# ChanganVR/RelationalGraphLearning

Hardware: AMD Instinct MI355X
Metric: agent-graph forward evals/sec (N=20, 2-layer GCN, depth-2 tree) (higher is better)
Workload: dtype f32 (24-bit operands throughout; 13 312 of the 14 224 products of the children kernel's 32 x 32, 32 x 100 and 100 x 100 head matrices, its embedding / graph weight products (w_r's second layer, Wa, W1, W_last) and the state predictor's weight products as six bf16 MFMA terms over three round-to-neare

## Files before the change

### relationalgraphlearning_amd/csrc/rgl_fused.hip

```cpp
#include "rgl_mlp_chain.h"
#include "rgl_scene_body.h"
#include "rgl_tail.h"

#include <mutex>
#include <unordered_map>
#include <vector>

namespace {

__host__ __device__ constexpr bool fused_packed_rows(int HR, bool SOFT) { return SOFT && HR <= 20; }
__host__ __device__ constexpr int fused_scratch_floats(int HR, int NT, bool SOFT) {
    const int NP = 16 * NT, HRL = HR < NP ? HR : NP;
    const int main_fl = fused_packed_rows(HR, SOFT) ? HRL * 32 + 16 * (HRL + 2) * 2 : 2 * 16 * (NP + 1) + 16 * XLD;
    const int crowd_fl = NP * XLD + 2 * NP;
    const int fl = main_fl > crowd_fl ? main_fl : crowd_fl;
    return ((fl > kTailLdsInts ? fl : kTailLdsInts) + 3) & ~3;
}

struct FusedArgs {
    const float *wr1, *br1, *wr2, *br2, *wa, *w1;
    const float *wh1, *bh1, *wh2, *bh2;
    const float* w_last;
    const float *hw1, *hb1, *hw2, *hb2, *hw3, *hb3, *hw4, *hb4;
    const float* child_robot;
// ... 237 lines not shown
                    xt[nt][ot][r] = Xs[(16 * nt + 4 * q + r) * XLD + 16 * ot + n];
        if constexpr (T1P) {
#pragma unroll
            for (int ot = 0; ot < 2; ++ot) xt1p[ot] = Xs[(16 + q) * XLD + 16 * ot + n];
        }
        load_fence();
        __builtin_amdgcn_wave_barrier();
        
        Split3 xqs[BX ? NT : 1], xts[BX ? 2 : 1];
        if constexpr (BX) {
            static_assert(NT <= 2, "Xh^T: one chunk over the nodes");
#pragma unroll
            for (int jt = 0; jt < NT; ++jt) xqs[jt] = split3_pair(xq[jt][0], xq[jt][1]);
            if constexpr (BXS) xpc[0] = xqs[0];
#pragma unroll
            for (int ft = 0; ft < 2; ++ft) xts[ft] = split3_pair(xt[0][ft], NT > 1 ? xt[NT > 1 ? 1 : 0][ft] : zero4());
        }
#pragma unroll
        for (int pct = 0; pct < NT; ++pct) {
            const int node = 16 * pct + n;
            const bool node_ok = node >= 1 && node < N;
            f32x4 e[NT];
            float mx = NEG_INF;
            Split3 gs;
            if constexpr (BX) {
                gs = split3_pair(gq[pct][0], gq[pct][1]);
                if (BXS && pct == 0) gpc[0] = gs;
            }
#pragma unroll
            for (int jt = 0; jt < NT; ++jt) {
                f32x4 sacc = zero4();
                if constexpr (BX) sacc = b6_block(xqs[jt], gs, sacc);
                else {
#pragma unroll
                for (int ft = 0; ft < 2; ++ft)
#pragma unroll
                    for (int r = 0; r < 4; ++r) sacc = mfma4(xq[jt][ft][r], gq[pct][ft][r], sacc);
                }
#pragma unroll
                for (int r = 0; r < 4; ++r) {
                    const int j = 16 * jt + 4 * q + r;
                    if (sim != SIM_SOFTMAX) sacc[r] = plain_weight(sim, sacc[r], node, j);
                    if (j < 1 || j >= N) sacc[r] = sim == SIM_SOFTMAX ? NEG_INF : 0.f;
                    mx = fmaxf(mx, sacc[r]);
                }
                e[jt] = sacc;
            }
            mx = kgroups_max(mx);
            if (!node_ok || sim != SIM_SOFTMAX) mx = 0.f;
            float z = 0.f;
#pragma unroll
            for (int jt = 0; jt < NT; ++jt)
#pragma unroll
                for (int r = 0; r < 4; ++r) {
                    if (sim == SIM_SOFTMAX) e[jt][r] = __expf(e[jt][r] - mx);
                    if (!node_ok) e[jt][r] = 0.f;
                    z += e[jt][r];
                }
            z = kgroups_sum(z);
            if (q == 0) {
                msz[node] = mx;
                msz[NP + node] = node_ok ? z : 1.f;
            }
            f32x4 u[2] = {zero4(), zero4()};
            f32x4 uw[2] = {zero4(), zero4()};
            {
            if constexpr (BX) {
                const Split3 es = split3_pair(e[0], NT > 1 ? e[NT > 1 ? 1 : 0] : zero4());
                u[0] = b6_block(xts[0], es, u[0]);
                u[1] = b6_block(xts[1], es, u[1]);
            } else {
#pragma unroll
            for (int jt = 0; jt < NT; ++jt)
#pragma unroll
                for (int r = 0; r < 4; ++r) {
                    u[0] = mfma4(xt[jt][0][r], e[jt][r], u[0]);
                    u[1] = mfma4(xt[jt][1][r], e[jt][r], u[1]);
                }
            }
            if constexpr (BX) layer_mfma_b6<XD, XD, false>(w1, u, uw, lane);
            else {
#pragma unroll
            for (int ft = 0; ft < 2; ++ft) {
                load_fence();
#pragma unroll
                for (int r = 0; r < 4; ++r)
#pragma unroll
                    for (int ot = 0; ot < 2; ++ot)
                        uw[ot] = mfma4(w1[(16 * ft + 4 * q + r) * WLD + 16 * ot + n], u[ft][r], uw[ot]);
            }
            load_fence();
            }
            }
            if constexpr (PK) {
                if (node < HRL) {
                    *reinterpret_cast<f32x4*>(&UWs[node * 32 + 4 * q]) = uw[0];
                    *reinterpret_cast<f32x4*>(&UWs[node * 32 + 16 + 4 * q]) = uw[1];
                }
            } else {
                *reinterpret_cast<f32x4*>(&Xs[node * XLD + 4 * q]) = uw[0];
                *reinterpret_cast<f32x4*>(&Xs[node * XLD + 16 + 4 * q]) = uw[1];
            }
        }
        __builtin_amdgcn_wave_barrier();
        load_fence();
#pragma unroll
        for (int nt = 0; nt < (T1P ? 1 : NT); ++nt) {
            ms[nt] = *reinterpret_cast<const f32x4*>(&msz[16 * nt + 4 * q]);
            zs[nt] = *reinterpret_cast<const f32x4*>(&msz[NP + 16 * nt + 4 * q]);
        }
        if constexpr (T1P) {
            ms1 = msz[16 + q];
            zs1 = msz[NP + 16 + q];
#pragma unroll
            for (int ot = 0; ot < 2; ++ot)
#pragma unroll
                for (int r = 0; r < 4; ++r) {
                    gq[1][ot][r] = quad0_bcast(gq[1][ot][r]);
                    xq[1][ot][r] = quad0_bcast(xq[1][ot][r]);
                }
        }
        if constexpr (!PK) {
#pragma unroll
            for (int i4 = 0; i4 < HRL / 4; ++i4)
#pragma unroll
                for (int k = 0; k < 4; ++k) uw4[i4][k] = Xs[(4 * i4 + k) * XLD + (lane & 31)];
        }
        load_fence();
        __builtin_amdgcn_wave_barrier();
    };
    static_assert(LO::scratch % 4 == 0 && LO::f_last % 4 == 0, "b128 granules");
    constexpr int kChunk = 256;
    constexpr int kChunksA = (LO::f_last + kChunk - 1) / kChunk, kChunksAll = (LO::scratch + kChunk - 1) / kChunk;
    int* image_arrivals = reinterpret_cast<int*>(lds + LO::scratch + kFusedWaves * fused_scratch_floats(HR, NT, SOFT));
    auto image_chunk = [&](int c) {
        const int fl = c * kChunk + lane * 4;
        if (fl < LO::scratch)
            __builtin_amdgcn_global_load_lds((const __attribute__((address_space(1))) void*)(a.image + fl),
                                             (__attribute__((address_space(3))) void*)(lds + c * kChunk), 16, 0, 0);
    };
    if constexpr (PRO) {
        static_assert(kPrologueSceneBase<LO> == kChunksA * kChunk, "the scene region starts behind the first part's chunks");
        static_assert(kPrologueSceneBase<LO> + prologue_scene_floats(2, 19) <= LO::scratch + kFusedWaves * fused_scratch_floats(HR, NT, SOFT) + 4,
                      "a two-layer predictor's scene region with the row buffer of a full chunk (12 crowds of 19 humans, 16 robot rows) fits the kernel's LDS");
        ProPhases pro_phases;
        ProPhases* const pp = &pro_phases;
        PRO_PHASE_START(pp);
        for (int c = wave; c < kChunksA; c += kFusedWaves) image_chunk(c);
#ifdef RGL_PROLOGUE_EMB_PER_WAVE
        constexpr bool kWge = false;
#else
        constexpr bool kWge = true;
#endif
        scene_body<2, 0, kFusedWaves, false, true, true, kWge>(pa.scene, lds + kPrologueSceneBase<LO>, p_first, 1, kFusedWaves,
                                                               p_first + k_b, pp);
        const ChildrenArgs& ca = pa.children;
        const long long pair0 = (long long)p_first * ca.A, pair_end = (long long)(p_first + k_b) * ca.A;
        if (ca.A >= 64 && ca.H <= 64 && !ca.robot64) {
            const float v_max = table_speed_bound(ca);
            for (long long base = pair0 + 64 * wave; base < pair_end; base += 64 * kFusedWaves) children_wave(ca, base, pair_end, v_max);
        } else {
            for (long long idx = pair0 + tid; idx < pair_end; idx += nthreads) children_thread(ca, idx);
        }
        PRO_PHASE_MARK(pp, 3);
        __syncthreads();
        PRO_PHASE_MARK(pp, 4);
        PRO_PHASE_FLUSH(pp);
        wh2_loads();
    }
    if (wave < n_items) item_loads(item_at(0));
    if (tid == 0) *image_arrivals = 0;
    bool image_complete = false;
    if (a.image_sync) {
        copy_image<LO::scratch, nthreads>(lds, a.image, tid);
        __syncthreads();
        image_complete = true;
    } else {
    if (!PRO) for (int c = wave; c < kChunksA; c += kFusedWaves) image_chunk(c);
    __builtin_amdgcn_s_waitcnt(0x0F70);
    __syncthreads();
    for (int c = kChunksA + wave; c < kChunksAll; c += kFusedWaves) image_chunk(c);
    }
    auto await_image = [&]() {
        if (image_complete) return;
        __builtin_amdgcn_s_waitcnt(0x0F70);
        asm volatile("" ::: "memory");
        if (lane == 0) __hip_atomic_fetch_add(image_arrivals, 1, __ATOMIC_RELEASE, __HIP_MEMORY_SCOPE_WORKGROUP);
        while (__hip_atomic_load(image_arrivals, __ATOMIC_ACQUIRE, __HIP_MEMORY_SCOPE_WORKGROUP) < kFusedWaves) __builtin_amdgcn_s_sleep(1);
        asm volatile("" ::: "memory");
        image_complete = true;
    };
    if (wave >= 4) {
        for (int i = 0; i < a.phase_delay; ++i) __builtin_amdgcn_s_sleep(8);
        if (a.prio & 1) __builtin_amdgcn_s_setprio(1);
    }
    PHASE_START();
    for (int pass = 0; pass < n_pass; ++pass) {
        const int wi = item_at(pass);
        if (wi >= n_items) break;
        const int wi_next = pass + 1 < n_pass ? item_at(pass + 1) : n_items;
        PHASE_MARK(0);
        int p, t0, ts, t1;
        item_tiles(wi, p, t0, ts, t1);
        load_fence();
        crowd_compute();
        PHASE_MARK(1);

      for (int ti = ts; ti < t1; ++ti) {
        const int t = ti < t0 ? a.n_full : ti;
        const bool full = t < a.n_full;
        const int c = 16 * t + n;
        const int n_valid = full ? 16 : a.rem;

        f32x4 xacc[2] = {zero4(), zero4()}, gacc[2] = {zero4(), zero4()}, yacc[2] = {zero4(), zero4()};
        float s00 = 0.f;
        Split3 sx;
        {
            f32x4 hacc[4] = {zero4(), zero4(), zero4(), zero4()};
#pragma unroll
            for (int s = 0; s < 3; ++s) {
                const int k = 4 * s + q;
#pragma unroll
                for (int ht = 0; ht < 4; ++ht) hacc[ht] = mfma4(wr1[(k < LO::WR1ROWS ? k : LO::WR1ROWS - 1) * LO::WR1LD + 16 * ht + n], rin[s], hacc[ht]);
            }
            if (ti + 1 < t1) robot_rows(p, ti + 1);
#pragma unroll
            for (int ht = 0; ht < 4; ++ht) {
                const f32x4 bb = *reinterpret_cast<const f32x4*>(&br1[16 * ht + 4 * q]);
#pragma unroll
                for (int r = 0; r < 4; ++r) hacc[ht][r] = relu1(hacc[ht][r] + bb[r]);
            }
            if constexpr (BX) {
                layer_mfma_b6<HID, XD, true>(wr2, hacc, xacc, lane, br2);
#pragma unroll
                for (int ot = 0; ot < 2; ++ot)
#pragma unroll
                    for (int r = 0; r < 4; ++r) xacc[ot][r] = relu1(xacc[ot][r]);
                sx = split3_pair(xacc[0], xacc[1]);
                layer_mfma_b6_pre<XD, false>(wa, sx, gacc, lane);
                layer_mfma_b6_pre<XD, false>(w1, sx, yacc, lane);
            } else {
#pragma unroll
            for (int ht = 0; ht < 4; ++ht) {
                load_fence();
#pragma unroll
                for (int r = 0; r < 4; ++r)
#pragma unroll
                    for (int ot = 0; ot < 2; ++ot)
                        xacc[ot] = mfma4(wr2[(16 * ht + 4 * q + r) * WLD + 16 * ot + n], hacc[ht][r], xacc[ot]);
            }
            load_fence();
#pragma unroll
            for (int ot = 0; ot < 2; ++ot) {
                const f32x4 bb = *reinterpret_cast<const f32x4*>(&br2[16 * ot + 4 * q]);
#pragma unroll
                for (int r = 0; r < 4; ++r) xacc[ot][r] = relu1(xacc[ot][r] + bb[r]);
            }
#pragma unroll
            for (int ot = 0; ot < 2; ++ot) {
                load_fence();
#pragma unroll
                for (int r = 0; r < 4; ++r)
#pragma unroll
                    for (int gt = 0; gt < 2; ++gt) {
                        gacc[gt] = mfma4(wa[(16 * ot + 4 * q + r) * WLD + 16 * gt + n], xacc[ot][r], gacc[gt]);
                        yacc[gt] = mfma4(w1[(16 * ot + 4 * q + r) * WLD + 16 * gt + n], xacc[ot][r], yacc[gt]);
                    }
            }
            load_fence();
            }
            if constexpr (!PK) {
                *reinterpret_cast<f32x4*>(&Y0[n * XLD + 4 * q]) = yacc[0];
                *reinterpret_cast<f32x4*>(&Y0[n * XLD + 16 + 4 * q]) = yacc[1];
            }
#pragma unroll
            for (int tt = 0; tt < 2; ++tt)
#pragma unroll
                for (int r = 0; r < 4; ++r) s00 = fmaf(gacc[tt][r], xacc[tt][r], s00);
            s00 = kgroups_sum(s00);
        }

        PHASE_MARK(2);
        f32x4 t0h[2] = {zero4(), zero4()};
        float p00;
        {
            f32x4 s0t[NT], sct[NT];
            float mx0 = NEG_INF;
            float sc1 = NEG_INF, p1 = NEG_INF;
            if constexpr (T1P) {
                f32x4 psc[2] = {zero4(), zero4()}, ps0[2] = {zero4(), zero4()};
#pragma unroll
                for (int ot = 0; ot < 2; ++ot)
#pragma unroll
                    for (int r = 0; r < 4; ++r) {
                        psc[r & 1] = mfma4x4(gq[1][ot][r], xacc[ot][r], psc[r & 1]);
                        ps0[r & 1] = mfma4x4(xq[1][ot][r], gacc[ot][r], ps0[r & 1]);
                    }
                sc1 = kgroups_reduce_scatter(psc[0] + psc[1]);
                p1 = kgroups_reduce_scatter(ps0[0] + ps0[1]);
                if (16 + q >= N) { sc1 = NEG_INF; p1 = NEG_INF; }
                mx0 = p1;
            }
            Split3 sg;
            if constexpr (BXS) sg = split3_pair(gacc[0], gacc[1]);
#pragma unroll
            for (int nt = 0; nt < NTS; ++nt) {
                f32x4 sc = zero4(), s0 = zero4();
// ... 751 lines not shown
```

### relationalgraphlearning_amd/csrc/rgl_mlp_chain.h

```cpp
#pragma once
#include "rgl_mfma.h"

namespace {

template <int D>
struct Tiles { static constexpr int v = (D + 15) / 16; };

template <int D>
__device__ __forceinline__ int tile_feature(int t, int q, int r) {
    constexpr bool partial = (D % 16) != 0;
    return (partial && t == Tiles<D>::v - 1) ? 16 * t + 4 * r + q : 16 * t + 4 * q + r;
}
template <int D>
struct LastTileSteps { static constexpr int v = (D % 16) == 0 ? 4 : ((D % 16) + 3) / 4; };

template <int OUT>
struct Partial4 { static constexpr bool v = (OUT % 16) != 0 && (OUT % 16) <= 4; };
template <int OUT>
__device__ __forceinline__ int frag_out_feature(int ot, int l) {
    if (Partial4<OUT>::v && ot == Tiles<OUT>::v - 1) return 16 * ot + (l & 3);
    const int m = l & 15;
    return tile_feature<OUT>(ot, m >> 2, m & 3);
}
template <int IN, int OUT, int NTHR = 0>
// ... 361 lines not shown
        constexpr int cn = (st + 1) / NP, prn = (st + 1) % NP;
        __builtin_amdgcn_sched_barrier(0);
        if constexpr (WB == 2 && has_next) {
#pragma unroll
            for (int g = 0; g < 2; ++g)
#pragma unroll
                for (int pc = 0; pc < 3; ++pc) w[WB == 2 ? buf ^ 1 : 0][g][pc] = frag_at(cn, 2 * prn + g, pc);
        }
        if constexpr (WB == 1) {
#pragma unroll
            for (int g = 0; g < 2; ++g)
#pragma unroll
                for (int pc = 0; pc < 3; ++pc) w[0][g][pc] = frag_at(c, 2 * pr + g, pc);
        }
        const bf16x8 sh = __builtin_bit_cast(bf16x8, u32x4{H[0], H[1], H[2], H[3]}), sm = __builtin_bit_cast(bf16x8, u32x4{M[0], M[1], M[2], M[3]}),
                     sl = __builtin_bit_cast(bf16x8, u32x4{L[0], L[1], L[2], L[3]});
#define RGL_BX_TERM(WP, AP)                                                                                         \
    _Pragma("unroll") for (int g = 0; g < 2; ++g)                                                                   \
        out[2 * pr + g] = __builtin_amdgcn_mfma_f32_16x16x32_bf16(w[buf][g][WP], AP, out[2 * pr + g], 0, 0, 0);
        RGL_BX_TERM(2, sh)
        RGL_BX_TERM(1, sm)
        RGL_BX_TERM(0, sl)
        RGL_BX_TERM(1, sh)
        RGL_BX_TERM(0, sm)
        RGL_BX_TERM(0, sh)
#undef RGL_BX_TERM
        if constexpr (c + 1 < NC) {
            constexpr int u0 = (4 * pr) / NP, u1 = (4 * (pr + 1)) / NP;
            static_for<u0, u1>([&](auto uc) {
                constexpr int p = decltype(uc)::value;
                split3_unit(unit_of(c + 1, p), Hn_[p], Mn_[p], Ln_[p]);
            });
        }
        if constexpr (WB == 1) __builtin_amdgcn_sched_group_barrier(0x100, 6, 0);
        __builtin_amdgcn_sched_group_barrier(0x008, 1, 0);
        if constexpr (WB == 2) __builtin_amdgcn_sched_group_barrier(0x100, has_next ? 6 : 0, 0);
#pragma unroll
        for (int i = 0; i < 11; ++i) {
            __builtin_amdgcn_sched_group_barrier(0x002, 2, 0);
            __builtin_amdgcn_sched_group_barrier(0x008, 1, 0);
        }
        if constexpr (pr == NP - 1 && c + 1 < NC) {
#pragma unroll
            for (int p = 0; p < 4; ++p) { H[p] = Hn_[p]; M[p] = Mn_[p]; L[p] = Ln_[p]; }
        }
    });
    __builtin_amdgcn_sched_barrier(0);
#pragma unroll
    for (int it = ITB + (BL::OT3 > 0 ? 2 : 0); it < IT; ++it) {
        load_fence();
#pragma unroll
        for (int r = 0; r < 4; ++r) {
            if (it == IT - 1 && r >= LastTileSteps<IN>::v) continue;
#pragma unroll
            for (int ot = 0; ot < OTF; ++ot) {
                const int k = (it - ITB - (ot < BL::OT3 ? 2 : 0)) * 4 + r;
                out[ot] = mfma4(fl[BL::f32_of(ot) + k * 64], in[it][r], out[ot]);
            }
        }
    }
    load_fence();
    if constexpr (BL::P4) out[OTF] = f32x4{v4, 0.f, 0.f, 0.f};
}

template <int IN, int OUT, bool BIAS>
__device__ __forceinline__ void layer_mfma_bx1(const float* frags, const f32x4 (&in)[Tiles<IN>::v], f32x4 (&out)[Tiles<OUT>::v],
                                               int lane, const float* bias = nullptr) {
    using BL = Bx1Layout<IN, OUT>;
    constexpr int OTF = BL::OTF;
    const int q = lane >> 4;
    float v4 = 0.f;
    if constexpr (BL::P4) {
        v4 = partial4_compact<IN, BL::KP>(frags + BL::p4, in, lane);
        if constexpr (BIAS) v4 += bias[16 * OTF + 4 * q];
    }
#pragma unroll
    for (int ot = 0; ot < OTF; ++ot) {
        if constexpr (BIAS) out[ot] = *reinterpret_cast<const f32x4*>(&bias[16 * ot + 4 * q]);
        else out[ot] = zero4();
    }
    load_fence();
    const Split3 s = split3_pair(in[0], in[1]);
    constexpr int G = 2;
#pragma unroll
    for (int o0 = 0; o0 < OTF; o0 += G) {
        load_fence();
        bf16x8 w[G][3];
#pragma unroll
        for (int g = 0; g < G; ++g)
#pragma unroll
            for (int pc = 0; pc < 3; ++pc)
                if (o0 + g < OTF) w[g][pc] = *reinterpret_cast<const bf16x8*>(&frags[BL::b16 + (((o0 + g) * 3 + pc) * 64 + lane) * 4]);
#define RGL_BX_TERM(WP, AP)                                                                                         \
    _Pragma("unroll") for (int g = 0; g < G; ++g)                                                                   \
        if (o0 + g < OTF) out[o0 + g] = __builtin_amdgcn_mfma_f32_16x16x32_bf16(w[g][WP], s.AP, out[o0 + g], 0, 0, 0);
        RGL_BX_TERM(2, h)
        RGL_BX_TERM(1, m)
        RGL_BX_TERM(0, l)
        RGL_BX_TERM(1, h)
        RGL_BX_TERM(0, m)
        RGL_BX_TERM(0, h)
#undef RGL_BX_TERM
    }
    load_fence();
    if constexpr (BL::P4) out[OTF] = f32x4{v4, 0.f, 0.f, 0.f};
}

template <int IN, int OUT>
struct B6Floats { static constexpr int v = Tiles<OUT>::v * ((Tiles<IN>::v + 1) / 2) * 3 * 64 * 4; };

template <int IN, int OUT, bool BIAS>
__device__ __forceinline__ void layer_mfma_b6(const float* frags, const f32x4 (&in)[Tiles<IN>::v], f32x4 (&out)[Tiles<OUT>::v],
                                              int lane, const float* bias = nullptr) {
    constexpr int IT = Tiles<IN>::v, OT = Tiles<OUT>::v, NC = (IT + 1) / 2;
    static_assert(IN % 16 == 0, "full input tiles");
    const int q = lane >> 4;
#pragma unroll
    for (int ot = 0; ot < OT; ++ot) {
        if constexpr (BIAS) out[ot] = *reinterpret_cast<const f32x4*>(&bias[16 * ot + 4 * q]);
        else out[ot] = zero4();
    }
    constexpr int G = 2, NOB = (OT + G - 1) / G, NB = NC * NOB;
    bf16x8 w[2][G][3];
    auto load_block = [&](int b, int buf) {
        const int c = b / NOB, o0 = G * (b % NOB);
#pragma unroll
        for (int g = 0; g < G; ++g)
#pragma unroll
            for (int pc = 0; pc < 3; ++pc)
                if (o0 + g < OT) w[buf][g][pc] = *reinterpret_cast<const bf16x8*>(&frags[((((o0 + g) * NC + c) * 3 + pc) * 64 + lane) * 4]);
    };
    load_fence();
    load_block(0, 0);
    Split3 s;
    static_for<0, NB>([&](auto bc) {
        constexpr int b = decltype(bc)::value, c = b / NOB, o0 = G * (b % NOB), buf = b & 1;
        if constexpr (b % NOB == 0) s = split3_pair(in[2 * c], 2 * c + 1 < IT ? in[2 * c + 1 < IT ? 2 * c + 1 : 0] : zero4());
        load_fence();
        if constexpr (b + 1 < NB) load_block(b + 1, buf ^ 1);
#define RGL_B6_TERM(WP, AP)                                                                                         \
    _Pragma("unroll") for (int g = 0; g < G; ++g)                                                                   \
        if (o0 + g < OT) out[o0 + g] = __builtin_amdgcn_mfma_f32_16x16x32_bf16(w[buf][g][WP], s.AP, out[o0 + g], 0, 0, 0);
        RGL_B6_TERM(2, h)
        RGL_B6_TERM(1, m)
        RGL_B6_TERM(0, l)
        RGL_B6_TERM(1, h)
        RGL_B6_TERM(0, m)
        RGL_B6_TERM(0, h)
#undef RGL_B6_TERM
    });
    load_fence();
}

template <int OUT, bool BIAS>
__device__ __forceinline__ void layer_mfma_b6_pre(const float* frags, const Split3& s, f32x4 (&out)[Tiles<OUT>::v], int lane,
                                                  const float* bias = nullptr) {
    constexpr int OT = Tiles<OUT>::v;
    const int q = lane >> 4;
#pragma unroll
    for (int ot = 0; ot < OT; ++ot) {
        if constexpr (BIAS) out[ot] = *reinterpret_cast<const f32x4*>(&bias[16 * ot + 4 * q]);
        else out[ot] = zero4();
    }
    constexpr int G = 2;
#pragma unroll
    for (int o0 = 0; o0 < OT; o0 += G) {
        load_fence();
        bf16x8 w[G][3];
#pragma unroll
        for (int g = 0; g < G; ++g)
#pragma unroll
            for (int pc = 0; pc < 3; ++pc)
                if (o0 + g < OT) w[g][pc] = *reinterpret_cast<const bf16x8*>(&frags[(((o0 + g) * 3 + pc) * 64 + lane) * 4]);
#define RGL_B6_TERM(WP, AP)                                                                                         \
    _Pragma("unroll") for (int g = 0; g < G; ++g)                                                                   \
        if (o0 + g < OT) out[o0 + g] = __builtin_amdgcn_mfma_f32_16x16x32_bf16(w[g][WP], s.AP, out[o0 + g], 0, 0, 0);
        RGL_B6_TERM(2, h)
        RGL_B6_TERM(1, m)
        RGL_B6_TERM(0, l)
        RGL_B6_TERM(1, h)
        RGL_B6_TERM(0, m)
        RGL_B6_TERM(0, h)
#undef RGL_B6_TERM
    }
    load_fence();
}

template <int IN, int OUT>
__device__ __forceinline__ float frag_bf3_ld(const float* __restrict__ W, int ld, int n_out, int idx) {
    constexpr int IT = Tiles<IN>::v, NC = (IT + 1) / 2;
    const int u = idx >> 2, p = idx & 3;
    const int l = u & 63, rest = u >> 6;
    const int pc = rest % 3, c = (rest / 3) % NC, ot = rest / 3 / NC;
    const int m = l & 15, q = l >> 4;
    const int out = 16 * ot + m;
    bf16x2 v;
#pragma unroll
    for (int k = 0; k < 2; ++k) {
        const int e = 2 * p + k, t = 2 * c + (e >> 2);
        const int in = 16 * t + 4 * q + (e & 3);
        const float w = (t < IT && in < IN && out < n_out) ? W[in * ld + out] : 0.f;
        const __bf16 hi = (__bf16)w;
        const float r1 = w - (float)hi;
        const __bf16 mid = (__bf16)r1;
        const __bf16 lo = (__bf16)(r1 - (float)mid);
        v[k] = pc == 0 ? hi : (pc == 1 ? mid : lo);
    }
    return __builtin_bit_cast(float, v);
}

template <int D>
__device__ __forceinline__ float frag_bf3_identity(int idx) {
    constexpr int IT = Tiles<D>::v, NC = (IT + 1) / 2;
    const int u = idx >> 2, p = idx & 3;
    const int l = u & 63, rest = u >> 6;
    const int pc = rest % 3, c = (rest / 3) % NC, ot = rest / 3 / NC;
    bf16x2 v;
#pragma unroll
    for (int k = 0; k < 2; ++k) {
        const int e = 2 * p + k, in = 16 * (2 * c + (e >> 2)) + 4 * (l >> 4) + (e & 3), out = 16 * ot + (l & 15);
        v[k] = (__bf16)((pc == 0 && in == out) ? 1.f : 0.f);
    }
    return __builtin_bit_cast(float, v);
}

template <int OUT>
__device__ __forceinline__ void relu_tiles(f32x4 (&x)[Tiles<OUT>::v]) {
#pragma unroll
    for (int ot = 0; ot < Tiles<OUT>::v; ++ot)
#pragma unroll
        for (int r = 0; r < 4; ++r) x[ot][r] = relu1(x[ot][r]);
}

}
```

### relationalgraphlearning_amd/csrc/rgl_scene_body.h

```cpp
#pragma once
#include "rgl_children.h"
#include "rgl_mlp_chain.h"

using rgl::LevelPrologue;
using rgl::SceneArgs;

namespace {

constexpr int M2LD = 20;

constexpr int kPrologueChunk = 16, kPrologueChunkCrowds = 12;
__host__ __device__ inline int prologue_chunk_end(int c0, int end, int crowds_per, int max_crowds) {
    int c1 = c0 + kPrologueChunk;
    const int by_crowds = (c0 / crowds_per + max_crowds) * crowds_per;
    if (by_crowds < c1) c1 = by_crowds;
    return c1 < end ? c1 : end;
}
constexpr int prologue_row_floats(int H, int max_crowds) { return (max_crowds * H + kPrologueChunk) * XD; }

struct SceneImageLayout { int off_wa, off_ws, off_wm1, off_bm1, off_wm2, off_bm2, total, ws_stride; };
constexpr SceneImageLayout scene_image_layout(int L, bool bx = false) {
    SceneImageLayout o{};
    int off = 0;
    auto take = [&](int nfl) { int r = off; off += (nfl + 3) & ~3; return r; };
    o.ws_stride = bx ? B6Floats<XD, XD>::v : XD * WLD;
    o.off_wa = take(bx ? B6Floats<XD, XD>::v : XD * WLD);
    o.off_ws = take(L * o.ws_stride);
    o.off_wm1 = take(bx ? B6Floats<XD, HID>::v : XD * W1LD);
    o.off_bm1 = take(HID);
    o.off_wm2 = take(bx ? B6Floats<HID, 16>::v : HID * M2LD);
    o.off_bm2 = take(16);
    o.total = off;
    return o;
}

constexpr int kRowMlpSetFloats = 4 * 1 * 4 * 64 + 2 * 4 * 4 * 64 + HID + XD;
constexpr int prologue_scene_floats(int L, int H) {
    return scene_image_layout(L, true).total + 2 * kRowMlpSetFloats + 8 * 32 * XLD + prologue_row_floats(H, kPrologueChunkCrowds);
}

#ifdef RGL_PHASE_TIMING
struct ProPhases { unsigned long long acc[5] = {0, 0, 0, 0, 0}, t0 = 0; };
#define PRO_PHASE_START(pp) do { if (pp) (pp)->t0 = __builtin_amdgcn_s_memtime(); } while (0)
#define PRO_PHASE_MARK(pp, idx)                                            \
    do {                                                                   \
        if (pp) {                                                          \
            const unsigned long long now__ = __builtin_amdgcn_s_memtime(); \
            (pp)->acc[idx] += now__ - (pp)->t0;                            \
            (pp)->t0 = now__;                                              \
        }                                                                  \
    } while (0)
#define PRO_PHASE_FLUSH(pp)                                                \
    do {                                                                   \
        if ((threadIdx.x & 63) == 0)                                       \
            for (int i__ = 0; i__ < 5; ++i__) atomicAdd(&g_phase_cycles[10 + i__], (pp)->acc[i__]); \
    } while (0)
#else
struct ProPhases {};
#define PRO_PHASE_START(pp) do { } while (0)
#define PRO_PHASE_MARK(pp, idx) do { } while (0)
#define PRO_PHASE_FLUSH(pp) do { (void)(pp); } while (0)
#endif

template <int IN>
__device__ __forceinline__ void row_mlp2_tile(const float* lds_set, const float* src, int lane, f32x4 (&o)[2]) {
    constexpr int F1 = 0, F2 = F1 + 4 * 1 * 4 * 64, B1 = F2 + 2 * 4 * 4 * 64, B2 = B1 + HID;
    const int q = lane >> 4;
    f32x4 in[1];
#pragma unroll
    for (int r = 0; r < 4; ++r) {
        const int feat = tile_feature<IN>(0, q, r);
        in[0][r] = feat < IN ? src[feat] : 0.f;
    }
    f32x4 h[4];
    layer_mfma<IN, HID, true>(lds_set + F1, in, h, lane, lds_set + B1);
    relu_tiles<HID>(h);
    layer_mfma<HID, XD, true>(lds_set + F2, h, o, lane, lds_set + B2);
    relu_tiles<XD>(o);
}


template <int NT, int SK, int WAVES, bool SPLIT, bool EMB = false, bool BX = false, bool WGE = false>
__device__ __forceinline__ void scene_body(const SceneArgs& a, float* lds, int first, int slot_step, int pass_step, int end,
                                           ProPhases* pp = nullptr) {
    static_assert(!BX || SK == 0, "six-term bf16 products: softmax similarity");
    static_assert(!WGE || (EMB && !SPLIT), "workgroup-cooperative embeddings: the embedding sets in LDS, one scene per wave");
    static_assert(!SPLIT || (SK != 3 && NT > 1 && WAVES % NT == 0), "split scenes: whole scenes per workgroup, no pair-MLP similarity");
    constexpr int kSceneThreads = WAVES * 64;
    constexpr int NCT = SPLIT ? 1 : NT;
    const int sim = SK == 0 ? (int)SIM_SOFTMAX : a.sim;
    const int tid = threadIdx.x, lane = tid & 63, wave = tid >> 6;
    const int n = lane & 15, q = lane >> 4;
    const int N = a.N, H = a.H;
    const float* wa = lds + a.off_wa;
    const float* ws = lds + a.off_ws;
    const float* wm1 = lds + a.off_wm1;
    const float* bm1 = lds + a.off_bm1;
    const float* wm2 = lds + a.off_wm2;
    const float* bm2 = lds + a.off_bm2;
    const int slot = __builtin_amdgcn_readfirstlane(SPLIT ? wave / NT : wave);
    const int ctb = SPLIT ? __builtin_amdgcn_readfirstlane(wave % NT) : 0;
    float* Hs = lds + a.off_wave + slot * a.wave_stride;
    constexpr int kEmbThreads = EMB ? kSceneThreads : 64;
    FragRegs<9, HID, kEmbThreads> er1;
    FragRegs<HID, XD, kEmbThreads> er2, eh2;
    FragRegs<5, HID, kEmbThreads> eh1;
    float ebias[4] = {0.f, 0.f, 0.f, 0.f};
    auto emb_loads = [&]() {
        if constexpr (EMB) {
            frag_load(er1, a.er_w1, tid);
            frag_load(er2, a.er_w2, tid);
            frag_load(eh1, a.eh_w1, tid);
            frag_load(eh2, a.eh_w2, tid);
            ebias[0] = bias_load<HID>(a.er_b1, tid);
            ebias[1] = bias_load<XD>(a.er_b2, tid);
            ebias[2] = bias_load<HID>(a.eh_b1, tid);
            ebias[3] = bias_load<XD>(a.eh_b2, tid);
        }
    };
    if constexpr (BX) {
        constexpr int kChunk = 256;
        const int n_chunks = (a.image_floats + kChunk - 1) / kChunk;
        for (int c = wave; c < n_chunks; c += WAVES) {
            const int fl = c * kChunk + lane * 4;
            if (fl < a.image_floats)
                __builtin_amdgcn_global_load_lds((const __attribute__((address_space(1))) void*)(a.image + fl),
                                                 (__attribute__((address_space(3))) void*)(lds + c * kChunk), 16, 0, 0);
        }
        __builtin_amdgcn_s_waitcnt(0x0F70);
    } else
    {
        float* w = lds;
        constexpr int NT_ = kSceneThreads;
        constexpr int KQ = XD * XD / NT_, KM1 = XD * HID / NT_, KM2 = HID * 16 / NT_;
        float vq[5][KQ];
        float vm1[KM1], vm2[KM2], vb;
        const int Lc = a.L < 4 ? a.L : 4;
#pragma unroll
        for (int k = 0; k < KQ; ++k) {
            const int i = tid + k * NT_;
            vq[0][k] = a.wa ? a.wa[i] : ((i / XD) == (i % XD) ? 1.f : 0.f);
#pragma unroll
            for (int l = 0; l < 4; ++l) vq[1 + l][k] = l < Lc ? a.Ws[l][i] : 0.f;
        }
#pragma unroll
        for (int k = 0; k < KM1; ++k) vm1[k] = a.wm1 ? a.wm1[tid + k * NT_] : 0.f;
#pragma unroll
        for (int k = 0; k < KM2; ++k) {
            const int i = tid + k * NT_, r = i / 16, c = i - r * 16;
            vm2[k] = a.wm2 ? a.wm2[r * 5 + (c < 5 ? c : 0)] : 0.f;
        }
        vb = !a.bm1 ? 0.f : (tid < HID ? a.bm1[tid] : (tid < HID + 5 ? a.bm2[tid - HID] : 0.f));
        emb_loads();
#pragma unroll
        for (int k = 0; k < KQ; ++k) {
            const int i = tid + k * NT_, r = i / XD, c = i - r * XD;
            w[a.off_wa + r * WLD + c] = vq[0][k];
#pragma unroll
            for (int l = 0; l < 4; ++l)
                if (l < Lc) w[a.off_ws + (l * XD + r) * WLD + c] = vq[1 + l][k];
        }
#pragma unroll
        for (int k = 0; k < KM1; ++k) {
            const int i = tid + k * NT_, r = i / HID, c = i - r * HID;
            w[a.off_wm1 + r * W1LD + c] = vm1[k];
        }
#pragma unroll
        for (int k = 0; k < KM2; ++k) {
            const int i = tid + k * NT_, r = i / 16, c = i - r * 16;
            w[a.off_wm2 + r * M2LD + c] = c < 5 ? vm2[k] : 0.f;
        }
        if (tid < HID) w[a.off_bm1 + tid] = vb;
        else if (tid < HID + 16) w[a.off_bm2 + tid - HID] = tid < HID + 5 ? vb : 0.f;
        if (SK == 3) {
            fill_matrix<2 * XD, 2 * XD, HID, W1LD, kSceneThreads>(w + a.off_wc1, a.wc1, tid);
            for (int i = tid; i < HID; i += kSceneThreads) { w[a.off_bc1 + i] = a.bc1[i]; w[a.off_wc2 + i] = a.wc2[i]; }
        }
    }
    if constexpr (EMB) {
        float* w = lds;
        constexpr int F1 = 0, F2 = F1 + 4 * 1 * 4 * 64, B1 = F2 + 2 * 4 * 4 * 64, B2 = B1 + HID;
        if constexpr (BX) emb_loads();
        frag_store(er1, w + a.off_er + F1, tid);
        frag_store(er2, w + a.off_er + F2, tid);
        bias_store<HID>(ebias[0], w + a.off_er + B1, tid);
        bias_store<XD>(ebias[1], w + a.off_er + B2, tid);
        frag_store(eh1, w + a.off_eh + F1, tid);
        frag_store(eh2, w + a.off_eh + F2, tid);
        bias_store<HID>(ebias[2], w + a.off_eh + B1, tid);
        bias_store<XD>(ebias[3], w + a.off_eh + B2, tid);
    }
    __syncthreads();
    PRO_PHASE_MARK(pp, 0);
    if (WGE && first >= end) return;
    int c0 = first;
    do {
    const int c1 = WGE ? prologue_chunk_end(c0, end, a.crowds_per, a.chunk_crowds) : end;
    const int cr0 = WGE ? c0 / a.crowds_per : 0;
    const int robot_rows0 = WGE ? a.off_rows + a.chunk_crowds * H * XD : 0;
    if constexpr (WGE) {
        if (c0 != first) {
            __syncthreads();
            PRO_PHASE_MARK(pp, 4);
        }
        const int hrows = ((c1 - 1) / a.crowds_per - cr0 + 1) * H, htiles = (hrows + 15) >> 4;
        for (int t = wave; t <= htiles; t += WAVES) {
            f32x4 o[2];
            int dst;
            bool valid;
            if (t < htiles) {
                const int row = 16 * t + n;
                valid = row < hrows;
                row_mlp2_tile<5>(lds + a.off_eh, a.human_rows + ((size_t)cr0 * H + (valid ? row : hrows - 1)) * 5, lane, o);
                dst = a.off_rows + row * XD;
            } else {
                valid = n < c1 - c0;
                row_mlp2_tile<9>(lds + a.off_er, a.robot_rows + (size_t)(valid ? c0 + n : c1 - 1) * 9, lane, o);
                dst = robot_rows0 + n * XD;
            }
            if (valid) {
                *reinterpret_cast<f32x4*>(&lds[dst + 4 * q]) = o[0];
                *reinterpret_cast<f32x4*>(&lds[dst + 16 + 4 * q]) = o[1];
            }
        }
        PRO_PHASE_MARK(pp, 1);
        __syncthreads();
        PRO_PHASE_MARK(pp, 4);
    }
    for (int it = c0 + (SPLIT ? 0 : slot_step * slot); it < c1; it += pass_step) {
        const int sc_raw = SPLIT ? it + slot_step * slot : it;
        const bool active = sc_raw < c1;
        const int sc = active ? sc_raw : c1 - 1;
        if constexpr (EMB && !WGE) {
            constexpr int F1 = 0, F2 = F1 + 4 * 1 * 4 * 64, B1 = F2 + 2 * 4 * 4 * 64, B2 = B1 + HID;
            const float* er = lds + a.off_er;
            const float* eh = lds + a.off_eh;
#pragma unroll
            for (int ct = 0; ct < NCT; ++ct) {
                const int node = 16 * (ct + ctb) + n;
                const bool human = node >= 1 && node < N;
                const float* hsrc = a.human_rows + ((size_t)(sc / a.crowds_per) * H + (human ? node - 1 : 0)) * 5;
                f32x4 in[1];
#pragma unroll
                for (int r = 0; r < 4; ++r) {
                    const int feat = tile_feature<5>(0, q, r);
                    in[0][r] = (human && feat < 5) ? hsrc[feat] : 0.f;
                }
                f32x4 hh[4], oh[2];
                layer_mfma<5, HID, true>(eh + F1, in, hh, lane, eh + B1);
                relu_tiles<HID>(hh);
                layer_mfma<HID, XD, true>(eh + F2, hh, oh, lane, eh + B2);
                relu_tiles<XD>(oh);
                if (ct + ctb == 0) {
                    const float* rsrc = a.robot_rows + (size_t)sc * 9;
#pragma unroll
                    for (int r = 0; r < 4; ++r) {
                        const int feat = tile_feature<9>(0, q, r);
                        in[0][r] = (n == 0 && feat < 9) ? rsrc[feat] : 0.f;
                    }
                    f32x4 orr[2];
                    layer_mfma<9, HID, true>(er + F1, in, hh, lane, er + B1);
                    relu_tiles<HID>(hh);
                    layer_mfma<HID, XD, true>(er + F2, hh, orr, lane, er + B2);
                    relu_tiles<XD>(orr);
                    if (n == 0) { oh[0] = orr[0]; oh[1] = orr[1]; }
                }
#pragma unroll
                for (int ot = 0; ot < 2; ++ot)
                    *reinterpret_cast<f32x4*>(&Hs[node * XLD + 16 * ot + 4 * q]) = node < N ? oh[ot] : zero4();
            }
            __builtin_amdgcn_wave_barrier();
        } else if constexpr (WGE) {
        const int xr = robot_rows0 + (sc - c0) * XD;
        const int xh = a.off_rows + (sc / a.crowds_per - cr0) * H * XD;
        for (int idx = lane; idx < 16 * NCT * (XD / 4); idx += 64) {
            const int row = (idx >> 3) + 16 * ctb, c4 = (idx & 7) * 4;
            f32x4 val = zero4();
            if (row == 0) val = *reinterpret_cast<const f32x4*>(&lds[xr + c4]);
            else if (row < N) val = *reinterpret_cast<const f32x4*>(&lds[xh + (row - 1) * XD + c4]);
            *reinterpret_cast<f32x4*>(&Hs[row * XLD + c4]) = val;
        }
        __builtin_amdgcn_wave_barrier();
        } else {
        const float* xr = a.x0_rows + (size_t)sc * XD;
        const float* xh = a.xh_rows + (size_t)(sc / a.crowds_per) * H * XD;
        for (int idx = lane; idx < 16 * NCT * (XD / 4); idx += 64) {
            const int row = (idx >> 3) + 16 * ctb, c4 = (idx & 7) * 4;
            f32x4 val = zero4();
            if (row == 0) val = *reinterpret_cast<const f32x4*>(xr + c4);
            else if (row < N) val = *reinterpret_cast<const f32x4*>(xh + (size_t)(row - 1) * XD + c4);
            *reinterpret_cast<f32x4*>(&Hs[row * XLD + c4]) = val;
        }
        }
        PRO_PHASE_MARK(pp, 1);
        if (SPLIT) __syncthreads();
        constexpr bool PERM = SK != 3;
        auto jnode = [&](int jt, int r) { return 16 * jt + ((PERM && jt == NT - 1) ? 4 * r + q : 4 * q + r); };
        const int last_steps = PERM ? (N - 16 * (NT - 1) + 3) >> 2 : 4;
        f32x4 pr[NT][NT];
        auto adjacency = [&]() {
            if constexpr (SK == 3) {
                const float* wc1 = lds + a.off_wc1;
                const float* bc1 = lds + a.off_bc1;
                const float* wc2 = lds + a.off_wc2;
                const float bc2 = a.bc2[0];
                f32x4 pt[NT][4], qt[NT][4];
#pragma unroll
                for (int ct = 0; ct < NT; ++ct) {
#pragma unroll
                    for (int ht = 0; ht < 4; ++ht) {
                        pt[ct][ht] = *reinterpret_cast<const f32x4*>(&bc1[16 * ht + 4 * q]);
                        qt[ct][ht] = zero4();
                    }
#pragma unroll
                    for (int ft = 0; ft < 2; ++ft) {
                        load_fence();
                        const f32x4 xb = *reinterpret_cast<const f32x4*>(&Hs[(16 * ct + n) * XLD + 16 * ft + 4 * q]);
#pragma unroll
                        for (int r = 0; r < 4; ++r)
#pragma unroll
                            for (int ht = 0; ht < 4; ++ht) {
                                pt[ct][ht] = mfma4(wc1[(16 * ft + 4 * q + r) * W1LD + 16 * ht + n], xb[r], pt[ct][ht]);
                                qt[ct][ht] = mfma4(wc1[(XD + 16 * ft + 4 * q + r) * W1LD + 16 * ht + n], xb[r], qt[ct][ht]);
                            }
                    }
                }
                f32x4 w2h[4];
#pragma unroll
                for (int ht = 0; ht < 4; ++ht) w2h[ht] = *reinterpret_cast<const f32x4*>(&wc2[16 * ht + 4 * q]);
#pragma unroll
                for (int ct = 0; ct < NT; ++ct)
#pragma unroll
                    for (int jt = 0; jt < NT; ++jt) {
                        f32x4 res = zero4();
                        static_for<0, 16>([&](auto jc) {
                            constexpr int jl = decltype(jc)::value;
                            float acc = 0.f;
#pragma unroll
                            for (int ht = 0; ht < 4; ++ht)
#pragma unroll
                                for (int r = 0; r < 4; ++r)
                                    acc = fmaf(fmaxf(dpp_rowbcast_add<jl>(qt[jt][ht][r], pt[ct][ht][r]), 0.f), w2h[ht][r], acc);
                            acc = fmaxf(kgroups_sum(acc) + bc2, 0.f);
                            const int j = 16 * jt + jl;
                            if (j >= N || 16 * ct + n >= N) acc = 0.f;
                            if ((jl >> 2) == q) res[jl & 3] = acc;
                        });
                        pr[ct][jt] = res;
                    }
                return;
            }
            f32x4 gt_[NT][2];
            {
#pragma unroll
            for (int ct = 0; ct < NCT; ++ct) {
                if constexpr (BX) {
                    load_fence();
                    f32x4 xin[2];
#pragma unroll
                    for (int ft = 0; ft < 2; ++ft)
                        xin[ft] = *reinterpret_cast<const f32x4*>(&Hs[(16 * (ct + ctb) + n) * XLD + 16 * ft + 4 * q]);
                    layer_mfma_b6<XD, XD, false>(wa, xin, gt_[ct], lane);
                    continue;
                }
                gt_[ct][0] = zero4();
                gt_[ct][1] = zero4();
                load_fence();
#pragma unroll
                for (int ft = 0; ft < 2; ++ft) {
                    const f32x4 xb = *reinterpret_cast<const f32x4*>(&Hs[(16 * (ct + ctb) + n) * XLD + 16 * ft + 4 * q]);
#pragma unroll
                    for (int r = 0; r < 4; ++r)
#pragma unroll
                        for (int g = 0; g < 2; ++g)
                            gt_[ct][g] = mfma4(wa[(16 * ft + 4 * q + r) * WLD + 16 * g + n], xb[r], gt_[ct][g]);
                }
            }
#pragma unroll
            for (int ct = 0; ct < NCT; ++ct)
#pragma unroll
                for (int jt = 0; jt < NT; ++jt) {
                    load_fence();
                    f32x4 sacc = zero4();
#pragma unroll
                    for (int ft = 0; ft < 2; ++ft) {
                        const int jrow = (PERM && jt == NT - 1) ? 4 * (n & 3) + (n >> 2) : n;
                        const f32x4 xa = *reinterpret_cast<const f32x4*>(&Hs[(16 * jt + jrow) * XLD + 16 * ft + 4 * q]);
#pragma unroll
                        for (int r = 0; r < 4; ++r) sacc = mfma4(xa[r], gt_[ct][ft][r], sacc);
                    }
                    pr[ct][jt] = sacc;
                }
            }
            if (SK == 2) {
                load_fence();
#pragma unroll
                for (int ct = 0; ct < NCT; ++ct) {
                    float z = 0.f;
#pragma unroll
                    for (int jt = 0; jt < NT; ++jt)
#pragma unroll
                        for (int r = 0; r < 4; ++r) z = fmaf(pr[ct][jt][r], pr[ct][jt][r], z);
                    z = kgroups_sum(z);
                    const float im = (16 * (ct + ctb) + n < N && z > 0.f) ? 1.f / sqrtf(z) : 0.f;
                    if (q == 0) Hs[(16 * (ct + ctb) + n) * XLD + 32] = im;
#pragma unroll
                    for (int jt = 0; jt < NT; ++jt)
#pragma unroll
                        for (int r = 0; r < 4; ++r) pr[ct][jt][r] *= im;
                }
                if (SPLIT) __syncthreads(); else __builtin_amdgcn_wave_barrier();
                load_fence();
#pragma unroll
                for (int jt = 0; jt < NT; ++jt)
#pragma unroll
                    for (int r = 0; r < 4; ++r) {
                        const float imj = Hs[jnode(jt, r) * XLD + 32];
#pragma unroll
                        for (int ct = 0; ct < NCT; ++ct) pr[ct][jt][r] *= imj;
                    }
                if (sim == SIM_COSINE) return;
            }
#pragma unroll
            for (int ct = 0; ct < NCT; ++ct) {
                float mx = -INFINITY;
#pragma unroll
                for (int jt = 0; jt < NT; ++jt)
#pragma unroll
                    for (int r = 0; r < 4; ++r) {
                        const int j = jnode(jt, r);
                        float v = pr[ct][jt][r];
                        if (SK == 1) v = plain_weight(sim, v, 16 * (ct + ctb) + n, j);
                        if (j >= N) v = SK == 1 ? 0.f : -INFINITY;
                        mx = fmaxf(mx, v);
                        pr[ct][jt][r] = v;
                    }
                mx = kgroups_max(mx);
                float sum = 0.f;
#pragma unroll
                for (int jt = 0; jt < NT; ++jt)
#pragma unroll
                    for (int r = 0; r < 4; ++r) {
                        if (SK != 1) pr[ct][jt][r] = __expf(pr[ct][jt][r] - mx);
                        sum += pr[ct][jt][r];
                    }
                sum = kgroups_sum(sum);
                const float inv = __builtin_amdgcn_rcpf(sum);
#pragma unroll
                for (int jt = 0; jt < NT; ++jt)
#pragma unroll
                    for (int r = 0; r < 4; ++r) pr[ct][jt][r] *= inv;
            }
        };
        if (!a.layerwise) adjacency();
        for (int l = 0; l < a.L; ++l) {
            if (a.layerwise) adjacency();
            const bool last = (l == a.L - 1);
            const bool rows_only = last && a.rows_out != nullptr;
            f32x4 acc[NT][2];
#pragma unroll
            for (int ct = 0; ct < NCT; ++ct) {
                acc[ct][0] = zero4();
                acc[ct][1] = zero4();
            }
            {
#pragma unroll
            for (int jt = 0; jt < NT; ++jt) {
                load_fence();
#pragma unroll
                for (int r = 0; r < 4; ++r) {
                    if (PERM && jt == NT - 1 && r >= last_steps) continue;
                    const float a0 = Hs[jnode(jt, r) * XLD + n];
                    const float a1 = Hs[jnode(jt, r) * XLD + 16 + n];
#pragma unroll
                    for (int ct = 0; ct < NCT; ++ct) {
                        if (rows_only && ct + ctb > 0) continue;
                        acc[ct][0] = mfma4(a0, pr[ct][jt][r], acc[ct][0]);
                        acc[ct][1] = mfma4(a1, pr[ct][jt][r], acc[ct][1]);
                    }
                }
            }
            }
            if (SPLIT) __syncthreads();
            if (rows_only) {
                if (active && ctb == 0) {
                    float* out = a.rows_out + (size_t)sc * 64;
                    if (n == 0) {
                        *reinterpret_cast<f32x4*>(out + 4 * q) = acc[0][0];
                        *reinterpret_cast<f32x4*>(out + 16 + 4 * q) = acc[0][1];
                    }
                    if (lane < 8) *reinterpret_cast<f32x4*>(out + 32 + 4 * lane) = *reinterpret_cast<const f32x4*>(&Hs[4 * lane]);
                }
                break;
            }
            const float* wl = ws + l * a.ws_stride;
#pragma unroll
            for (int ct = 0; ct < NCT; ++ct) {
                load_fence();
                f32x4 o[2] = {zero4(), zero4()};
                if constexpr (BX) {
                    layer_mfma_b6<XD, XD, false>(wl, acc[ct], o, lane);
                } else {
#pragma unroll
                for (int ft = 0; ft < 2; ++ft)
#pragma unroll
                    for (int r = 0; r < 4; ++r)
#pragma unroll
                        for (int ot = 0; ot < 2; ++ot)
                            o[ot] = mfma4(wl[(16 * ft + 4 * q + r) * WLD + 16 * ot + n], acc[ct][ft][r], o[ot]);
                }
#pragma unroll
                for (int ot = 0; ot < 2; ++ot) {
                    const f32x4 sk = *reinterpret_cast<const f32x4*>(&Hs[(16 * (ct + ctb) + n) * XLD + 16 * ot + 4 * q]);
#pragma unroll
                    for (int r = 0; r < 4; ++r) {
                        float hv = fmaxf(o[ot][r], 0.f);
                        if (a.skip) hv += sk[r];
                        o[ot][r] = 16 * (ct + ctb) + n < N ? hv : 0.f;
                    }
                    if (!last) *reinterpret_cast<f32x4*>(&Hs[(16 * (ct + ctb) + n) * XLD + 16 * ot + 4 * q]) = o[ot];
                }
                if (last) {
                    f32x4 hm[4] = {zero4(), zero4(), zero4(), zero4()};
                    f32x4 om = zero4();
                    if constexpr (BX) {
                        layer_mfma_b6<XD, HID, true>(wm1, o, hm, lane, bm1);
#pragma unroll
                        for (int ht = 0; ht < 4; ++ht)
#pragma unroll
                            for (int r = 0; r < 4; ++r) hm[ht][r] = fmaxf(hm[ht][r], 0.f);
                        f32x4 om1[1];
                        layer_mfma_b6<HID, 16, false>(wm2, hm, om1, lane);
                        om = om1[0];
                    } else {
#pragma unroll
                    for (int ot = 0; ot < 2; ++ot) {
                        load_fence();
#pragma unroll
                        for (int r = 0; r < 4; ++r)
#pragma unroll
                            for (int ht = 0; ht < 4; ++ht)
                                hm[ht] = mfma4(wm1[(16 * ot + 4 * q + r) * W1LD + 16 * ht + n], o[ot][r], hm[ht]);
                    }
#pragma unroll
                    for (int ht = 0; ht < 4; ++ht) {
                        load_fence();
                        const f32x4 bb = *reinterpret_cast<const f32x4*>(&bm1[16 * ht + 4 * q]);
#pragma unroll
                        for (int r = 0; r < 4; ++r) {
                            const float hv = fmaxf(hm[ht][r] + bb[r], 0.f);
                            om = mfma4(wm2[(16 * ht + 4 * q + r) * M2LD + n], hv, om);
                        }
                    }
                    }
                    const int node = 16 * (ct + ctb) + n;
                    if (active && node >= 1 && node < N) {
                        float* dst = a.humans_next + ((size_t)sc * H + (node - 1)) * 5;
#pragma unroll
                        for (int r = 0; r < 4; ++r) {
                            const int oidx = 4 * q + r;
                            if (oidx < 5) dst[oidx] = om[r] + bm2[oidx];
                        }
                    }
                }
            }
            if (SPLIT) __syncthreads(); else __builtin_amdgcn_wave_barrier();
        }
        if (SPLIT) __syncthreads();
        PRO_PHASE_MARK(pp, 2);
    }
    c0 = c1;
    } while (WGE && c0 < end);
}

}
```

Baseline: 2.166 billion.

## Pipeline six-term bf16 layers across both node tiles in scene prologue

Adds a column-batched six-term bf16 MFMA layer routine that processes both 16-node tiles together. It double-buffers the weight fragments, interleaves the splitting of the next inputs with the current MFMAs, and uses scheduling group barriers. The prologue scene body now uses it for the Wa similarity transform, each GCN layer, and the state-predictor MLP, with fused per-tile epilogues. The embedding weight loads are also issued earlier, alongside the image loads. This aims to hide load and conversion latency behind MFMA work, at the cost of more registers and more complex code.

Result: no change. 2.172 billion (median of 6 runs) (+0.2%).

```diff
diff --git a/relationalgraphlearning_amd/csrc/rgl_fused.hip b/relationalgraphlearning_amd/csrc/rgl_fused.hip
--- a/relationalgraphlearning_amd/csrc/rgl_fused.hip
+++ b/relationalgraphlearning_amd/csrc/rgl_fused.hip
@@ -413,7 +413,7 @@
 #else
         constexpr bool kWge = true;
 #endif
-        scene_body<2, 0, kFusedWaves, false, true, true, kWge>(pa.scene, lds + kPrologueSceneBase<LO>, p_first, 1, kFusedWaves,
+        scene_body<2, 0, kFusedWaves, false, true, true, kWge, true>(pa.scene, lds + kPrologueSceneBase<LO>, p_first, 1, kFusedWaves,
                                                                p_first + k_b, pp);
         const ChildrenArgs& ca = pa.children;
         const long long pair0 = (long long)p_first * ca.A, pair_end = (long long)(p_first + k_b) * ca.A;
diff --git a/relationalgraphlearning_amd/csrc/rgl_mlp_chain.h b/relationalgraphlearning_amd/csrc/rgl_mlp_chain.h
--- a/relationalgraphlearning_amd/csrc/rgl_mlp_chain.h
+++ b/relationalgraphlearning_amd/csrc/rgl_mlp_chain.h
@@ -537,6 +537,82 @@
     load_fence();
 }
 
+template <int IN, int OUT, bool BIAS, int NCOL, class Epi>
+__device__ __forceinline__ void layer_mfma_b6_cols(const float* frags, const f32x4 (&in)[NCOL][Tiles<IN>::v],
+                                                   f32x4 (&out)[NCOL][Tiles<OUT>::v], int lane, const float* bias, Epi&& epi) {
+    constexpr int IT = Tiles<IN>::v, OT = Tiles<OUT>::v, NCH = IT / 2;
+    static_assert(IN % 32 == 0, "whole K = 32 chunks");
+    const int q = lane >> 4;
+#pragma unroll
+    for (int k = 0; k < NCOL; ++k)
+#pragma unroll
+        for (int ot = 0; ot < OT; ++ot) {
+            if constexpr (BIAS) out[k][ot] = *reinterpret_cast<const f32x4*>(&bias[16 * ot + 4 * q]);
+            else out[k][ot] = zero4();
+        }
+    constexpr int G = 2, NOB = (OT + G - 1) / G, NB = NCH * NOB, NS = NB * NCOL, NSP = NCH * NCOL;
+    bf16x8 w[2][G][3];
+    auto load_block = [&](int b, int buf) {
+        const int c = b / NOB, o0 = G * (b % NOB);
+#pragma unroll
+        for (int g = 0; g < G; ++g)
+#pragma unroll
+            for (int pc = 0; pc < 3; ++pc)
+                if (o0 + g < OT) w[buf][g][pc] = *reinterpret_cast<const bf16x8*>(&frags[((((o0 + g) * NCH + c) * 3 + pc) * 64 + lane) * 4]);
+    };
+    load_fence();
+    load_block(0, 0);
+    unsigned H[NSP][4], M[NSP][4], L[NSP][4];
+    auto unit_of = [&](int j, int p) {
+        const int k = j % NCOL, t = 2 * (j / NCOL) + (p >> 1), r0 = 2 * (p & 1);
+        return f32x2{in[k][t][r0], in[k][t][r0 + 1]};
+    };
+#pragma unroll
+    for (int p = 0; p < 4; ++p) split3_unit(unit_of(0, p), H[0][p], M[0][p], L[0][p]);
+    static_for<0, NS>([&](auto stc) {
+        constexpr int st = decltype(stc)::value, b = st / NCOL, k = st % NCOL, c = b / NOB, o0 = G * (b % NOB), buf = b & 1;
+        constexpr int j = c * NCOL + k, NG = OT - o0 < G ? OT - o0 : G;
+        constexpr bool loads = k == 0 && b + 1 < NB;
+        __builtin_amdgcn_sched_barrier(0);
+        if constexpr (loads) load_block(b + 1, buf ^ 1);
+        const bf16x8 sh = __builtin_bit_cast(bf16x8, u32x4{H[j][0], H[j][1], H[j][2], H[j][3]}),
+                     sm = __builtin_bit_cast(bf16x8, u32x4{M[j][0], M[j][1], M[j][2], M[j][3]}),
+                     sl = __builtin_bit_cast(bf16x8, u32x4{L[j][0], L[j][1], L[j][2], L[j][3]});
+#define RGL_B6_TERM(WP, AP)                                                                                         \
+    _Pragma("unroll") for (int g = 0; g < NG; ++g)                                                                  \
+        out[k][o0 + g] = __builtin_amdgcn_mfma_f32_16x16x32_bf16(w[buf][g][WP], AP, out[k][o0 + g], 0, 0, 0);
+        RGL_B6_TERM(2, sh)
+        RGL_B6_TERM(1, sm)
+        RGL_B6_TERM(0, sl)
+        RGL_B6_TERM(1, sh)
+        RGL_B6_TERM(0, sm)
+        RGL_B6_TERM(0, sh)
+#undef RGL_B6_TERM
+        static_for<1, NSP>([&](auto jc) {
+            constexpr int jn = decltype(jc)::value;
+            constexpr int lo = ((jn - 1) / NCOL) * NOB * NCOL + (jn - 1) % NCOL, hi = (jn / NCOL) * NOB * NCOL + jn % NCOL;
+            if constexpr (st >= lo && st < hi) {
+                constexpr int u0 = 4 * (st - lo) / (hi - lo), u1 = 4 * (st - lo + 1) / (hi - lo);
+                static_for<u0, u1>([&](auto uc) {
+                    constexpr int p = decltype(uc)::value;
+                    split3_unit(unit_of(jn, p), H[jn][p], M[jn][p], L[jn][p]);
+                });
+            }
+        });
+        if constexpr (b == NB - 1 && k >= 1) epi(std::integral_constant<int, k - 1>{});
+        __builtin_amdgcn_sched_group_barrier(0x008, 1, 0);
+        if constexpr (loads) __builtin_amdgcn_sched_group_barrier(0x100, 3 * (OT - G * ((b + 1) % NOB) < G ? OT - G * ((b + 1) % NOB) : G), 0);
+#pragma unroll
+        for (int i = 0; i < 6 * NG - 1; ++i) {
+            __builtin_amdgcn_sched_group_barrier(0x002, 2, 0);
+            __builtin_amdgcn_sched_group_barrier(0x008, 1, 0);
+        }
+    });
+    __builtin_amdgcn_sched_barrier(0);
+    epi(std::integral_constant<int, NCOL - 1>{});
+    load_fence();
+}
+
 template <int OUT, bool BIAS>
 __device__ __forceinline__ void layer_mfma_b6_pre(const float* frags, const Split3& s, f32x4 (&out)[Tiles<OUT>::v], int lane,
                                                   const float* bias = nullptr) {
diff --git a/relationalgraphlearning_amd/csrc/rgl_scene_body.h b/relationalgraphlearning_amd/csrc/rgl_scene_body.h
--- a/relationalgraphlearning_amd/csrc/rgl_scene_body.h
+++ b/relationalgraphlearning_amd/csrc/rgl_scene_body.h
@@ -80,10 +80,11 @@
 }
 
 
-template <int NT, int SK, int WAVES, bool SPLIT, bool EMB = false, bool BX = false, bool WGE = false>
+template <int NT, int SK, int WAVES, bool SPLIT, bool EMB = false, bool BX = false, bool WGE = false, bool COLS = false>
 __device__ __forceinline__ void scene_body(const SceneArgs& a, float* lds, int first, int slot_step, int pass_step, int end,
                                            ProPhases* pp = nullptr) {
     static_assert(!BX || SK == 0, "six-term bf16 products: softmax similarity");
+    static_assert(!COLS || (BX && !SPLIT && NT == 2), "column-tile pipeline: the unsplit six-term form over two node tiles");
     static_assert(!WGE || (EMB && !SPLIT), "workgroup-cooperative embeddings: the embedding sets in LDS, one scene per wave");
     static_assert(!SPLIT || (SK != 3 && NT > 1 && WAVES % NT == 0), "split scenes: whole scenes per workgroup, no pair-MLP similarity");
     constexpr int kSceneThreads = WAVES * 64;
@@ -127,6 +128,7 @@
                 __builtin_amdgcn_global_load_lds((const __attribute__((address_space(1))) void*)(a.image + fl),
                                                  (__attribute__((address_space(3))) void*)(lds + c * kChunk), 16, 0, 0);
         }
+        emb_loads();
         __builtin_amdgcn_s_waitcnt(0x0F70);
     } else
     {
@@ -180,7 +182,6 @@
     if constexpr (EMB) {
         float* w = lds;
         constexpr int F1 = 0, F2 = F1 + 4 * 1 * 4 * 64, B1 = F2 + 2 * 4 * 4 * 64, B2 = B1 + HID;
-        if constexpr (BX) emb_loads();
         frag_store(er1, w + a.off_er + F1, tid);
         frag_store(er2, w + a.off_er + F2, tid);
         bias_store<HID>(ebias[0], w + a.off_er + B1, tid);
@@ -351,7 +352,34 @@
                 return;
             }
             f32x4 gt_[NT][2];
-            {
+            if constexpr (COLS) {
+                load_fence();
+                f32x4 xin[NT][2];
+#pragma unroll
+                for (int ct = 0; ct < NT; ++ct)
+#pragma unroll
+                    for (int ft = 0; ft < 2; ++ft)
+                        xin[ct][ft] = *reinterpret_cast<const f32x4*>(&Hs[(16 * ct + n) * XLD + 16 * ft + 4 * q]);
+                layer_mfma_b6_cols<XD, XD, false, NT>(wa, xin, gt_, lane, nullptr, [](auto) {});
+#pragma unroll
+                for (int jt = 0; jt < NT; ++jt) {
+                    load_fence();
+                    f32x4 sacc[NT];
+#pragma unroll
+                    for (int ct = 0; ct < NT; ++ct) sacc[ct] = zero4();
+#pragma unroll
+                    for (int ft = 0; ft < 2; ++ft) {
+                        const int jrow = (PERM && jt == NT - 1) ? 4 * (n & 3) + (n >> 2) : n;
+                        const f32x4 xa = *reinterpret_cast<const f32x4*>(&Hs[(16 * jt + jrow) * XLD + 16 * ft + 4 * q]);
+#pragma unroll
+                        for (int ct = 0; ct < NT; ++ct)
+#pragma unroll
+                            for (int r = 0; r < 4; ++r) sacc[ct] = mfma4(xa[r], gt_[ct][ft][r], sacc[ct]);
+                    }
+#pragma unroll
+                    for (int ct = 0; ct < NT; ++ct) pr[ct][jt] = sacc[ct];
+                }
+            } else {
 #pragma unroll
             for (int ct = 0; ct < NCT; ++ct) {
                 if constexpr (BX) {
@@ -494,6 +522,51 @@
                 break;
             }
             const float* wl = ws + l * a.ws_stride;
+            if constexpr (COLS) {
+                f32x4 o[NT][2];
+                auto layer_epi = [&](auto kc, auto store) {
+                    constexpr int ct = decltype(kc)::value;
+                    const bool valid = 16 * ct + n < N;
+#pragma unroll
+                    for (int ot = 0; ot < 2; ++ot) {
+                        const f32x4 sk = *reinterpret_cast<const f32x4*>(&Hs[(16 * ct + n) * XLD + 16 * ot + 4 * q]);
+#pragma unroll
+                        for (int r = 0; r < 4; ++r) {
+                            const float hv = fmaxf(o[ct][ot][r], 0.f);
+                            o[ct][ot][r] = valid ? (a.skip ? hv + sk[r] : hv) : 0.f;
+                        }
+                        if constexpr (decltype(store)::value)
+                            *reinterpret_cast<f32x4*>(&Hs[(16 * ct + n) * XLD + 16 * ot + 4 * q]) = o[ct][ot];
+                    }
+                };
+                load_fence();
+                if (!last) {
+                    layer_mfma_b6_cols<XD, XD, false, NT>(wl, acc, o, lane, nullptr, [&](auto kc) { layer_epi(kc, std::true_type{}); });
+                } else {
+                    layer_mfma_b6_cols<XD, XD, false, NT>(wl, acc, o, lane, nullptr, [&](auto kc) { layer_epi(kc, std::false_type{}); });
+                    f32x4 hm[NT][4], om[NT][1];
+                    layer_mfma_b6_cols<XD, HID, true, NT>(wm1, o, hm, lane, bm1, [&](auto kc) {
+                        constexpr int ct = decltype(kc)::value;
+#pragma unroll
+                        for (int ht = 0; ht < 4; ++ht)
+#pragma unroll
+                            for (int r = 0; r < 4; ++r) hm[ct][ht][r] = fmaxf(hm[ct][ht][r], 0.f);
+                    });
+                    layer_mfma_b6_cols<HID, 16, false, NT>(wm2, hm, om, lane, nullptr, [](auto) {});
+#pragma unroll
+                    for (int ct = 0; ct < NT; ++ct) {
+                        const int node = 16 * ct + n;
+                        if (active && node >= 1 && node < N) {
+                            float* dst = a.humans_next + ((size_t)sc * H + (node - 1)) * 5;
+#pragma unroll
+                            for (int r = 0; r < 4; ++r) {
+                                const int oidx = 4 * q + r;
+                                if (oidx < 5) dst[oidx] = om[ct][0][r] + bm2[oidx];
+                            }
+                        }
+                    }
+                }
+            } else {
 #pragma unroll
             for (int ct = 0; ct < NCT; ++ct) {
                 load_fence();
@@ -564,6 +637,7 @@
                     }
                 }
             }
+            }
             if (SPLIT) __syncthreads(); else __builtin_amdgcn_wave_barrier();
         }
         if (SPLIT) __syncthreads();
```
